# dohlee/diffab-pytorch

Hardware: NVIDIA B200
Metric: reverse-diffusion patches/s (K=128, T=100) (higher is better)
Workload: dtype bf16

## Files before the change

### diffab-pytorch_b200/csrc/ipa_sm100.cu

```cuda
#include <cuda_bf16.h>
#include <cuda_fp16.h>

#include <stdlib.h>

#include <mutex>

#include "common.cuh"
#include "gemm_sm100.cuh"
#include "ipa_proj_sm100.cuh"
#include "ipa_sm100_layout.cuh"
#include "sm100_prims.cuh"

namespace dab {

EncodeTiledFn get_encode_tiled() {
  static EncodeTiledFn fn = nullptr;
  static std::once_flag once;
  std::call_once(once, [] {
    void* p = nullptr;
    cudaDriverEntryPointQueryResult q;
    if (cudaGetDriverEntryPoint("cuTensorMapEncodeTiled", &p, cudaEnableDefault, &q) == cudaSuccess &&
        q == cudaDriverEntryPointSuccess)
      fn = reinterpret_cast<EncodeTiledFn>(p);
  });
  return fn;
}

int make_tensor_map_bf16(CUtensorMap* out, const void* base, int rank, const uint64_t* dims,
                         const uint64_t* strides_bytes, const uint32_t* box, CUtensorMapSwizzle swizzle) {
  EncodeTiledFn enc = get_encode_tiled();
  DAB_REQUIRE(enc != nullptr, DAB_ELAUNCH, "cuTensorMapEncodeTiled not available (no CUDA driver?)");
  cuuint64_t gdim[5];
  cuuint64_t gstr[5];
  cuuint32_t bdim[5], estr[5];
  for (int i = 0; i < rank; ++i) { gdim[i] = dims[i]; bdim[i] = box[i]; estr[i] = 1; }
  for (int i = 0; i + 1 < rank; ++i) gstr[i] = strides_bytes[i];
  CUresult r = enc(out, CU_TENSOR_MAP_DATA_TYPE_BFLOAT16, (cuuint32_t)rank, const_cast<void*>(base), gdim, gstr, bdim,
                   estr, CU_TENSOR_MAP_INTERLEAVE_NONE, swizzle, CU_TENSOR_MAP_L2_PROMOTION_L2_128B,
                   CU_TENSOR_MAP_FLOAT_OOB_FILL_NONE);
  DAB_REQUIRE(r == CUDA_SUCCESS, DAB_EINVAL, "cuTensorMapEncodeTiled failed with CUresult %d", (int)r);
  return DAB_OK;
}

namespace sm100 {

#ifdef DAB_DEBUG_HOOKS
static long long* g_core_dbg = nullptr;
#else
static constexpr long long* g_core_dbg = nullptr;
#endif

__global__ void __launch_bounds__(256) pack_weights_kernel(DabIpaWeights w, uint8_t* packed) {
  __shared__ float tile[32][33];
  const PackedOffsets o = packed_offsets();
  constexpr int kCatTiles = (NPROJ / 32) * (D / 32);
  const int tx = threadIdx.x & 31, ty = threadIdx.x >> 5;
  const float* src;
  __nv_bfloat16 *dst, *dst_t;
  int r0, c0, ld_src, ld_dst, ld_t, row_off = 0;
  int t = blockIdx.x;
  if (t < kCatTiles) {
    const int tr = t / (D / 32), tcn = t % (D / 32);
    r0 = tr * 32; c0 = tcn * 32;
    const float* srcs[6] = {w.w_q_scalar, w.w_k_scalar, w.w_v_scalar, w.w_q_point, w.w_k_point, w.w_v_point};
    const int seg = r0 < 3 * NS ? r0 / NS : 3 + (r0 - 3 * NS) / NPT;
    row_off = seg < 3 ? seg * NS : 3 * NS + (seg - 3) * NPT;
    src = srcs[seg]; ld_src = D;
    dst = reinterpret_cast<__nv_bfloat16*>(packed + o.wcat); ld_dst = D;
    dst_t = reinterpret_cast<__nv_bfloat16*>(packed + o.wcat_t); ld_t = NPROJ;
  } else {
    t -= kCatTiles;
    const int tr = t / (NCAT / 32), tcn = t % (NCAT / 32);
    r0 = tr * 32; c0 = tcn * 32;
    src = w.w_out; ld_src = NCAT;
    dst = reinterpret_cast<__nv_bfloat16*>(packed + o.wout); ld_dst = NCAT;
    dst_t = reinterpret_cast<__nv_bfloat16*>(packed + o.wout_t); ld_t = D;
  }
#pragma unroll
  for (int k = 0; k < 4; ++k) {
    const int r = ty + 8 * k;
    const float v = __ldg(src + (size_t)(r0 - row_off + r) * ld_src + c0 + tx);
    tile[r][tx] = v;
    dst[(size_t)(r0 + r) * ld_dst + c0 + tx] = __float2bfloat16_rn(v);
  }
  __syncthreads();
#pragma unroll
  for (int k = 0; k < 4; ++k) {
    const int c = ty + 8 * k;
    dst_t[(size_t)(c0 + c) * ld_t + r0 + tx] = __float2bfloat16_rn(tile[tx][c]);
  }
  if (blockIdx.x == 0) {
    float* wpb = reinterpret_cast<float*>(packed + o.wpb);
    for (int i = threadIdx.x; i < H * C; i += 256) wpb[i] = w.w_pair_bias[i];
    float* bout = reinterpret_cast<float*>(packed + o.bout);
    float* gam = reinterpret_cast<float*>(packed + o.gamma);
    for (int i = threadIdx.x; i < D; i += 256) bout[i] = w.b_out[i];
    for (int i = threadIdx.x; i < H; i += 256) gam[i] = w.gamma[i];
  }
}
constexpr int kPackBlocks = (NPROJ / 32) * (D / 32) + (D / 32) * (NCAT / 32);

struct CoreSmem {
  static constexpr int kSlot = L * C * 2;
  static constexpr int kSlots = 4;
  static constexpr int kRing = 0;
  static constexpr int kKBuf = 3 * L * 64;
  static constexpr int kKBufs = 3;
  static constexpr int kKRing = kRing + kSlots * kSlot;
  static constexpr int kCtx0 = kKRing + kKBufs * kKBuf;
  static constexpr int kPh = 0;
  static constexpr int kPhBytes = H * 2 * IB * 128;
  static constexpr int kQBuf = H * 3 * IB * 64;
  static constexpr int kPi = kPh + kPhBytes;
  static constexpr int kPiSlot = 2 * 2048;
  static constexpr int kCtxBytes = kPi + 2 * kPiSlot;
  static constexpr int kMisc = kCtx0 + 2 * kCtxBytes;
  static constexpr int kRedMax = kMisc;
  static constexpr int kBars = kRedMax + 2 * 1024;
  static constexpr int kNumBars = 48;
  static constexpr int kTmemSlot = kBars + kNumBars * 8;
  static constexpr int kTotal = kTmemSlot + 16;
};
static_assert(CoreSmem::kQBuf <= CoreSmem::kPhBytes, "Q must fit the idle P_h region");
static_assert(CoreSmem::kTotal <= 227 * 1024, "one CTA per SM");

enum Bar { K_FULL = 0, K_EMPTY = 3, R_FULL = 6, R_EMPTY = 10, K_TURN = 14, R_TURN = 15, CTX_BARS = 16, N_BARS = 16 + 2 * 13 };
enum CtxBar { Q_FULL = 0, S_DONE = 1, PAIR = 2 , O_DONE = 4, P_READY = 5 ,
              EPI_TMEM = 9 ,
              EPI_DONE = 10 ,
              EPI_SFREE = 11 , N_CTX_BARS = 13 };
static_assert(N_BARS <= CoreSmem::kNumBars, "barrier storage");

constexpr uint32_t kColS = 0, kColPair = 128 , kTmemCols = 512;

template <bool IS_MAX>
__device__ __forceinline__ float warp_reduce8(const float (&v)[8], int lane) {
  auto op = [](float a, float b) { return IS_MAX ? fmaxf(a, b) : a + b; };
  const bool u1 = lane & 16, u2 = lane & 8, u3 = lane & 4;
  float a[4], bq[2];
#pragma unroll
  for (int k = 0; k < 4; ++k) {
    float send = u1 ? v[k] : v[k + 4], keep = u1 ? v[k + 4] : v[k];
    a[k] = op(keep, __shfl_xor_sync(0xffffffffu, send, 16));
  }
#pragma unroll
  for (int k = 0; k < 2; ++k) {
    float send = u2 ? a[k] : a[k + 2], keep = u2 ? a[k + 2] : a[k];
    bq[k] = op(keep, __shfl_xor_sync(0xffffffffu, send, 8));
  }
  float send = u3 ? bq[0] : bq[1], keep = u3 ? bq[1] : bq[0];
  float c = op(keep, __shfl_xor_sync(0xffffffffu, send, 4));
  c = op(c, __shfl_xor_sync(0xffffffffu, c, 2));
  c = op(c, __shfl_xor_sync(0xffffffffu, c, 1));
  return c;
}

__device__ __forceinline__ float warp_reduce16_max(const float (&v)[16], int lane) {
  const bool u1 = lane & 16, u2 = lane & 8, u3 = lane & 4, u4 = lane & 2;
  float a[8], b4[4], c2[2];
#pragma unroll
  for (int k = 0; k < 8; ++k) {
    float send = u1 ? v[k] : v[k + 8], keep = u1 ? v[k + 8] : v[k];
    a[k] = fmaxf(keep, __shfl_xor_sync(0xffffffffu, send, 16));
  }
#pragma unroll
  for (int k = 0; k < 4; ++k) {
    float send = u2 ? a[k] : a[k + 4], keep = u2 ? a[k + 4] : a[k];
    b4[k] = fmaxf(keep, __shfl_xor_sync(0xffffffffu, send, 8));
  }
#pragma unroll
  for (int k = 0; k < 2; ++k) {
    float send = u3 ? b4[k] : b4[k + 2], keep = u3 ? b4[k + 2] : b4[k];
    c2[k] = fmaxf(keep, __shfl_xor_sync(0xffffffffu, send, 4));
  }
  float send = u4 ? c2[0] : c2[1], keep = u4 ? c2[1] : c2[0];
  float d = fmaxf(keep, __shfl_xor_sync(0xffffffffu, send, 2));
  return fmaxf(d, __shfl_xor_sync(0xffffffffu, d, 1));
}

__device__ __forceinline__ void tmem_ld_x4(uint32_t taddr, float (&v)[4]) {
  uint32_t r[4];
  asm volatile("tcgen05.ld.sync.aligned.32x32b.x4.b32 {%0,%1,%2,%3}, [%4];"
               : "=r"(r[0]), "=r"(r[1]), "=r"(r[2]), "=r"(r[3])
               : "r"(taddr));
#pragma unroll
  for (int i = 0; i < 4; ++i) v[i] = __uint_as_float(r[i]);
}

constexpr int kCoreThreads = 640;
template <bool KB2>
__global__ void __launch_bounds__(kCoreThreads, 1)
ipa_core_kernel(const __grid_constant__ CUtensorMap map_q, const __grid_constant__ CUtensorMap map_k,
                const __grid_constant__ CUtensorMap map_v, const __grid_constant__ CUtensorMap map_e,
                const uint4* __restrict__ bias, const float* __restrict__ tc, const float* __restrict__ R,
                __nv_bfloat16* __restrict__ cat, float* __restrict__ stats, uint4* __restrict__ pu,
                int n_tiles, long long* __restrict__ dbg, int64_t out_stride) {
  extern __shared__ __align__(1024) uint8_t smem[];
  long long* dbg_cta = nullptr;
#define DAB_STAMP(k) do { if (dbg_cta && (threadIdx.x & 255) == 0) dbg_cta[(k)] = clock64(); } while (0)
#define DAB_STAMP_ISSUER(k) do { if (dbg_cta) dbg_cta[(k)] = clock64(); } while (0)
#define DAB_TIMED_WAIT(bar, par, acc) do { if (dbg) { long long t0_ = clock64(); mbar_wait((bar), (par)); (acc) += clock64() - t0_; } else mbar_wait((bar), (par)); } while (0)
  using S = CoreSmem;
  uint64_t* bars = reinterpret_cast<uint64_t*>(smem + S::kBars);
  uint32_t* tmem_slot = reinterpret_cast<uint32_t*>(smem + S::kTmemSlot);

  const int tid = threadIdx.x, warp = tid >> 5, lane = tid & 31;
  const uint32_t smem_base = smem_u32(smem);
  if ((smem_base & 1023u) != 0) asm volatile("trap;");
  const int n_local = (n_tiles - (int)blockIdx.x + (int)gridDim.x - 1) / (int)gridDim.x;
  auto tile_of = [&](int k) { return n_tiles - 1 - ((int)blockIdx.x + k * (int)gridDim.x); };
  struct TileIdx { int64_t q0, kv0, o0; int lrow, joff; };
  auto decode = [&](int tile) {
    TileIdx ti;
    const int v = tile >> 3, it = tile & 7;
    if (KB2) {
      const int qblk = v >> 1, kb = v & 1;
      ti.q0 = (int64_t)qblk * L + it * IB;
      ti.kv0 = (int64_t)((qblk & ~1) + kb) * L;
      ti.o0 = (int64_t)kb * out_stride + ti.q0;
      ti.lrow = 2 * L; ti.joff = kb * L;
    } else {
      ti.q0 = (int64_t)v * L + it * IB; ti.kv0 = (int64_t)v * L; ti.o0 = ti.q0; ti.lrow = L; ti.joff = 0;
    }
    return ti;
  };
  auto pos_e = [](int r) { return r; };
  auto pos_v = [](int h) { return IB + h; };
  auto k_use = [](int k, int h) { return k * (h % 3 == 2 ? 2 : 3) + h / 3; };

  if (tid == 0) {
    for (int i = 0; i < CTX_BARS; ++i) mbar_init(&bars[i], 1u);
    for (int c = 0; c < 2; ++c)
      for (int i = 0; i < N_CTX_BARS; ++i)
        mbar_init(&bars[CTX_BARS + N_CTX_BARS * c + i], (i >= P_READY && i < P_READY + 4) ? 128u : (i >= EPI_TMEM ? 256u : 1u));
    fence_barrier_init();
  }
  __syncwarp();
  if (warp == 0) tmem_alloc(tmem_slot, kTmemCols);
  tcgen05_fence_before_sync();
  __syncthreads();
  tcgen05_fence_after_sync();
  const uint32_t tmem_cta = *tmem_slot;

  if (warp == 18) {
    if (lane == 0) {
      tma_prefetch_desc(&map_q); tma_prefetch_desc(&map_k);
      for (int k = 0; k < n_local; ++k) {
        const int c = k & 1, n = k >> 1, tile = tile_of(k);
        const TileIdx ti = decode(tile);
        const int64_t row0 = ti.q0;
        const int kvrow = (int)ti.kv0;
        uint64_t* cb = bars + CTX_BARS + N_CTX_BARS * c;
        uint8_t* cs = smem + S::kCtx0 + c * S::kCtxBytes;
        auto load_k = [&](int h) {
          const int s = h % S::kKBufs;
          if (k > 0 || h >= S::kKBufs) mbar_wait(&bars[K_EMPTY + s], (k_use(k, h) - 1) & 1);
          uint8_t* kb = smem + S::kKRing + s * S::kKBuf;
          mbar_arrive_expect_tx(&bars[K_FULL + s], S::kKBuf);
          for (int blk = 0; blk < 3; ++blk)
            tma_load_2d(kb + blk * (L * 64), &map_k, &bars[K_FULL + s], (h * 3 + blk) * 32, kvrow);
        };
        load_k(0);
        load_k(1);
        load_k(2);
        if (n > 0) mbar_wait(&cb[O_DONE], (n - 1) & 1);
        mbar_arrive_expect_tx(&cb[Q_FULL], S::kQBuf);
        for (int blk = 0; blk < H * 3; ++blk)
          tma_load_2d(cs + S::kPh + blk * (IB * 64), &map_q, &cb[Q_FULL], blk * 32, (int)row0);
        for (int h = S::kKBufs; h < H; ++h) load_k(h);
      }
    }
  } else if (warp == 19) {
    if (lane == 0) {
      tma_prefetch_desc(&map_v); tma_prefetch_desc(&map_e);
      const uint64_t pol = policy_evict_first();
#ifndef DAB_L2_AHEAD
#define DAB_L2_AHEAD 8
#endif
      constexpr int kL2Ahead = DAB_L2_AHEAD;
      auto pair0_of = [&](int k, int r) { const TileIdx ti = decode(tile_of(k)); return (int)((ti.q0 + r) * ti.lrow + ti.joff); };
      if (n_local > 0)
        for (int r = 0; r < kL2Ahead; ++r) tma_prefetch_l2_2d_hint(&map_e, 0, pair0_of(0, r), pol);
      for (int k = 0; k < n_local; ++k) {
        const int kvrow = (int)decode(tile_of(k)).kv0;
        const bool has_next = k + 1 < n_local;
        for (int x = 0; x < IB + H; ++x) {
          const int s = x % S::kSlots;
          if (k > 0 || x >= S::kSlots) mbar_wait(&bars[R_EMPTY + s], ((x / S::kSlots) + 1) & 1);
          mbar_arrive_expect_tx(&bars[R_FULL + s], S::kSlot);
          if (x < IB) {
            tma_load_2d_hint(smem + S::kRing + s * S::kSlot, &map_e, &bars[R_FULL + s], 0, pair0_of(k, x), pol);
            const int a = x + kL2Ahead;
            if (a < IB) tma_prefetch_l2_2d_hint(&map_e, 0, pair0_of(k, a), pol);
            else if (has_next) tma_prefetch_l2_2d_hint(&map_e, 0, pair0_of(k + 1, a - IB), pol);
          } else {
            tma_load_2d(smem + S::kRing + s * S::kSlot, &map_v, &bars[R_FULL + s], (x - IB) * V_W, kvrow);
          }
        }
      }
    }
  } else if (warp >= 16) {
    const int c = __shfl_sync(0xffffffffu, warp, 0) - 16;
    {
      constexpr uint32_t kIdescS = make_idesc_bf16(128, 16, 0, 0);
      constexpr uint32_t kIdescPair = make_idesc_bf16(128, 16, 1, 0);
      constexpr uint32_t kIdescO = make_idesc_f16(128, 32, 1, 0);
      uint64_t* cb = bars + CTX_BARS + N_CTX_BARS * c;
      const uint32_t cs = smem_base + S::kCtx0 + c * S::kCtxBytes;
      const uint32_t tmem = tmem_cta + 256u * c;
      const uint64_t dK0 = make_smem_desc(smem_base + S::kKRing, 16, 512, kSwizzle64B);
      const uint64_t dQ0 = make_smem_desc(cs + S::kPh, 16, 512, kSwizzle64B);
      const uint64_t dR0 = make_smem_desc(smem_base + S::kRing, S::kSlot, 1024, kSwizzle128B);
      const uint64_t dPi0 = make_smem_desc(cs + S::kPi, 16, 1024, kSwizzle128B);
      const uint64_t dPh0 = make_smem_desc(cs + S::kPh, 16, 1024, kSwizzle128B);
      for (int k = c, n = 0; k < n_local; k += 2, ++n) {
        dbg_cta = (dbg && lane == 0) ? dbg + (size_t)tile_of(k) * 64 : nullptr;
        long long w_q = 0, w_sfree = 0, w_kturn = 0, w_k = 0, w_epit = 0, w_rturn = 0, w_e = 0, w_p = 0, w_v = 0;
        DAB_STAMP_ISSUER(16);
        DAB_TIMED_WAIT(&cb[Q_FULL], n & 1, w_q);
        if (n > 0) {
          DAB_TIMED_WAIT(&cb[EPI_SFREE], (n - 1) & 1, w_sfree);
        }
        if (k > 0) DAB_TIMED_WAIT(&bars[K_TURN], (k - 1) & 1, w_kturn);
        tcgen05_fence_after_sync();
        DAB_STAMP_ISSUER(1);
        for (int h = 0; h < H; ++h) {
          const int s = h % S::kKBufs;
          DAB_TIMED_WAIT(&bars[K_FULL + s], k_use(k, h) & 1, w_k);
          tcgen05_fence_after_sync();
          DAB_STAMP_ISSUER(48 + h);
          if (elect_one()) {
            const uint64_t ka = dK0 + (uint32_t)((s * S::kKBuf) >> 4);
            const uint64_t qa = dQ0 + (uint32_t)((h * 3 * (IB * 64)) >> 4);
#pragma unroll
            for (int m = 0; m < 4; ++m) {
              const int ablk = (m == 0) ? 0 : (m == 3 ? 2 : 1), bblk = (m == 0) ? 0 : (m == 2 ? 2 : 1);
#pragma unroll
              for (int kk = 0; kk < 2; ++kk)
                umma_bf16(tmem + kColS + h * 16, ka + (uint32_t)((ablk * (L * 64) + kk * 32) >> 4),
                          qa + (uint32_t)((bblk * (IB * 64) + kk * 32) >> 4), kIdescS, (m | kk) != 0);
            }
            umma_commit(&bars[K_EMPTY + s]);
          }
          __syncwarp();
        }
        if (elect_one()) {
          umma_commit(&cb[S_DONE]);
          mbar_arrive(&bars[K_TURN]);
        }
        __syncwarp();
        DAB_STAMP_ISSUER(2);
        if (n > 0) DAB_TIMED_WAIT(&cb[EPI_TMEM], (n - 1) & 1, w_epit);
        if (k > 0) DAB_TIMED_WAIT(&bars[R_TURN], (k - 1) & 1, w_rturn);
        DAB_STAMP_ISSUER(17);
        for (int p = 0; p < IB / 2; ++p) {
          const int x = pos_e(2 * p), st = x % S::kSlots;
          const int slot = p & 1;
          DAB_TIMED_WAIT(&bars[R_FULL + st], (x / S::kSlots) & 1, w_e);
          DAB_TIMED_WAIT(&bars[R_FULL + st + 1], (x / S::kSlots) & 1, w_e);
          if (p == 4) DAB_STAMP_ISSUER(41);
          DAB_TIMED_WAIT(&cb[P_READY + slot], (p >> 1) & 1, w_p);
          DAB_TIMED_WAIT(&cb[P_READY + 2 + slot], (p >> 1) & 1, w_p);
          tcgen05_fence_after_sync();
          if (p == 4) DAB_STAMP_ISSUER(42);
          if (elect_one()) {
            const uint64_t ea = dR0 + (uint32_t)((st * S::kSlot) >> 4);
            const uint64_t pa = dPi0 + (uint32_t)((slot * S::kPiSlot) >> 4);
#pragma unroll
            for (int kk = 0; kk < L / 16; ++kk)
              umma_bf16(tmem + kColPair + p * 16, ea + (uint32_t)((kk * 2048) >> 4),
                        pa + (uint32_t)(((kk >> 2) * 2048 + (kk & 3) * 32) >> 4), kIdescPair, kk != 0);
            umma_commit(&cb[PAIR + slot]);
            umma_commit(&bars[R_EMPTY + st]);
            umma_commit(&bars[R_EMPTY + st + 1]);
          }
          __syncwarp();
          if (p == 4) DAB_STAMP_ISSUER(43);
        }
        DAB_STAMP_ISSUER(3);
        for (int m = 0; m < H / 2; ++m) {
          const int x = pos_v(2 * m), st = x % S::kSlots;
          DAB_TIMED_WAIT(&bars[R_FULL + st], (x / S::kSlots) & 1, w_v);
          DAB_TIMED_WAIT(&bars[R_FULL + st + 1], (x / S::kSlots) & 1, w_v);
          tcgen05_fence_after_sync();
          DAB_STAMP_ISSUER(56 + m);
          if (elect_one()) {
            const uint64_t va = dR0 + (uint32_t)((st * S::kSlot) >> 4);
            const uint64_t pa = dPh0 + (uint32_t)(((2 * m) * (IB * 128)) >> 4);
#pragma unroll
            for (int kk = 0; kk < L / 16; ++kk)
              umma_bf16(tmem + kColS + m * 32, va + (uint32_t)((kk * 2048) >> 4),
                        pa + (uint32_t)(((kk >> 2) * (H * IB * 128) + (kk & 3) * 32) >> 4), kIdescO, kk != 0);
            umma_commit(&bars[R_EMPTY + st]);
            umma_commit(&bars[R_EMPTY + st + 1]);
          }
          __syncwarp();
        }
        if (elect_one()) {
          umma_commit(&cb[O_DONE]);
          mbar_arrive(&bars[R_TURN]);
        }
        __syncwarp();
        DAB_STAMP_ISSUER(7);
        if (dbg_cta) {
          dbg_cta[18] = w_q; dbg_cta[19] = w_sfree; dbg_cta[20] = w_kturn; dbg_cta[21] = w_k; dbg_cta[22] = w_epit;
          dbg_cta[23] = w_rturn; dbg_cta[25] = w_e; dbg_cta[26] = w_p; dbg_cta[27] = w_v;
        }
      }
    }
  } else {
    const int c = warp >> 3, cw = warp & 7;
    const int g = cw >> 2, gw = cw & 3, gt = tid & 127, ct = tid & 255;
    uint64_t* cb = bars + CTX_BARS + N_CTX_BARS * c;
    uint8_t* cs = smem + S::kCtx0 + c * S::kCtxBytes;
    const uint32_t tmem = tmem_cta + 256u * c;
    const uint32_t tmem_lane = tmem + ((uint32_t)(gw * 32) << 16);
    const int vsel = ((lane >> 4) & 1) * 8 + ((lane >> 3) & 1) * 4 + ((lane >> 2) & 1) * 2 + ((lane >> 1) & 1);
    float* red_max = reinterpret_cast<float*>(smem + S::kRedMax) + c * 256 + g * 128;
    float* red_ctx = reinterpret_cast<float*>(smem + S::kRedMax) + c * 256;
    float* inv_o = red_ctx;
    auto bar_group = [&] { asm volatile("bar.sync %0, 128;" ::"r"(1 + 2 * c + g) : "memory"); };
    auto bar_all_compute = [&] { asm volatile("bar.sync %0, 256;" ::"r"(5 + c) : "memory"); };
    (void)ct;

   for (int k = c, tn = 0; k < n_local; k += 2, ++tn) {
    const int tile = tile_of(k);
    const TileIdx ti = decode(tile);
    const int64_t row0 = ti.q0;
    const int64_t orow0 = KB2 ? ti.o0 : row0;
    constexpr int64_t LR = KB2 ? 2 * L : L;
    dbg_cta = dbg ? dbg + (size_t)tile * 64 : nullptr;
    long long w_pair = 0;
    DAB_STAMP(0);
    const uint4* bias_t = bias + (row0 + g) * LR + (KB2 ? ti.joff : 0) + gt;
    uint4 b_cur[2] = {__ldg(bias_t), __ldg(bias_t + 2 * LR)};
    uint4 b_nxt[2] = {__ldg(bias_t + 4 * LR), __ldg(bias_t + 6 * LR)};
    mbar_wait(&cb[S_DONE], tn & 1);
    tcgen05_fence_after_sync();
    DAB_STAMP(6);
    for (int q = 0; q < IB / 4; ++q) {
      const uint4 b_use[2] = {b_cur[0], b_cur[1]};
      b_cur[0] = b_nxt[0]; b_cur[1] = b_nxt[1];
      if (q + 2 < IB / 4) {
        b_nxt[0] = __ldg(bias_t + (size_t)(2 * q + 4) * 2 * LR);
        b_nxt[1] = __ldg(bias_t + (size_t)(2 * q + 5) * 2 * LR);
      }
      float sreg[H][4];
#pragma unroll
      for (int h = 0; h < H; ++h) tmem_ld_x4(tmem_lane + kColS + h * 16 + 4 * q, sreg[h]);
      tmem_wait_ld();
      if (q == IB / 4 - 1) tcgen05_fence_before_sync();
      if (q == 2) DAB_STAMP(33);
      float lg[16];
#pragma unroll
      for (int r = 0; r < 2; ++r) {
        const __half2* hb = reinterpret_cast<const __half2*>(&b_use[r]);
#pragma unroll
        for (int kk = 0; kk < 4; ++kk) {
          float2 f = __half22float2(hb[kk]);
          lg[r * 8 + 2 * kk] = f.x; lg[r * 8 + 2 * kk + 1] = f.y;
        }
#pragma unroll
        for (int h = 0; h < H; ++h) {
          const float sv = g == 0 ? (r == 0 ? sreg[h][0] : sreg[h][2]) : (r == 0 ? sreg[h][1] : sreg[h][3]);
          lg[r * 8 + h] += sv;
        }
      }
      float wm = warp_reduce16_max(lg, lane);
      float* rm = red_max + (q & 1) * 64;
      if ((lane & 1) == 0) rm[gw * 16 + vsel] = wm;
      bar_group();
      if (q == 2) DAB_STAMP(34);
      float mx[16];
      {
        const float4* r4 = reinterpret_cast<const float4*>(rm);
#pragma unroll
        for (int kk = 0; kk < 4; ++kk) {
          float4 a = r4[kk], bb = r4[4 + kk], cc = r4[8 + kk], dd = r4[12 + kk];
          mx[4 * kk] = fmaxf(fmaxf(a.x, bb.x), fmaxf(cc.x, dd.x));
          mx[4 * kk + 1] = fmaxf(fmaxf(a.y, bb.y), fmaxf(cc.y, dd.y));
          mx[4 * kk + 2] = fmaxf(fmaxf(a.z, bb.z), fmaxf(cc.z, dd.z));
          mx[4 * kk + 3] = fmaxf(fmaxf(a.w, bb.w), fmaxf(cc.w, dd.w));
        }
      }
      if (stats && gt < 16) {
        float v = mx[0];
#pragma unroll
        for (int kk = 1; kk < 16; ++kk) v = (kk == gt) ? mx[kk] : v;
        stats[(orow0 + 2 * (2 * q + (gt >> 3)) + g) * 16 + (gt & 7)] = v;
      }
#pragma unroll
      for (int r = 0; r < 2; ++r) {
        const int n = 2 * q + r, i = 2 * n + g;
        float p[8];
#pragma unroll
        for (int h = 0; h < H; ++h) p[h] = ex2(lg[r * 8 + h] - mx[r * 8 + h]);
        if (pu)
          pu[(row0 + i) * L + gt] = make_uint4(pack_bf162(p[0], p[1]), pack_bf162(p[2], p[3]), pack_bf162(p[4], p[5]),
                                               pack_bf162(p[6], p[7]));
        if (n >= 2) DAB_TIMED_WAIT(&cb[PAIR + (n & 1)], ((n >> 1) - 1) & 1, w_pair);
        {
          const int je = gt & ~1;
          const uint32_t kb = je >> 6, chunk = (je & 63) >> 3, e2 = (je & 7) * 2;
          uint8_t* pi = cs + S::kPi + (n & 1) * S::kPiSlot + kb * 2048 + g * 1024;
          uint8_t* ph = cs + S::kPh + kb * (H * IB * 128);
          const bool odd = lane & 1;
#pragma unroll
          for (int hh = 0; hh < 4; ++hh) {
            float send = odd ? p[2 * hh] : p[2 * hh + 1];
            float recv = __shfl_xor_sync(0xffffffffu, send, 1);
            const int h = 2 * hh + (odd ? 1 : 0);
            float lo = odd ? recv : p[2 * hh], hi = odd ? p[2 * hh + 1] : recv;
            *reinterpret_cast<uint32_t*>(pi + swz128_offset(h, chunk) + e2) = pack_bf162(lo, hi);
            *reinterpret_cast<uint32_t*>(ph + h * (IB * 128) + swz128_offset(i, chunk) + e2) = pack_h2(lo, hi);
          }
        }
        fence_proxy_async_smem();
        tcgen05_fence_before_sync();
        mbar_arrive(&cb[P_READY + g * 2 + (n & 1)]);
        if (g == 0) DAB_STAMP(8 + n);
      }
    }
    DAB_STAMP(24);
    if (dbg_cta && (tid & 255) == 0) dbg_cta[28] = w_pair;

    float Rm[9], tfr[3];
    {
      const int64_t row = row0 + (gt >> 3);
#pragma unroll
      for (int cc = 0; cc < 9; ++cc) Rm[cc] = __ldg(R + row * 9 + cc);
#pragma unroll
      for (int cc = 0; cc < 3; ++cc) tfr[cc] = __ldg(tc + row * 3 + cc);
    }
    uint8_t* stage_e = cs + S::kPh + S::kQBuf + 12288 + cw * 512;
    mbar_wait(&cb[O_DONE], tn & 1);
    tcgen05_fence_after_sync();
    DAB_STAMP(4);
    const int hsel = gw >> 1;
    const uint32_t ocol = kColS + (uint32_t)hsel * 16;
    if (gw & 1) {
#pragma unroll
      for (int mm = 0; mm < 2; ++mm) {
        const int m = 2 * g + mm, h = 2 * m + hsel;
        float o[16];
        tmem_ld_x16(tmem_lane + ocol + m * 32, o);
        tmem_wait_ld();
        if (lane == 24) {
#pragma unroll
          for (int i = 0; i < IB; ++i) inv_o[i * H + h] = __fdividef(1.0f, o[i]);
        }
      }
    }
    bar_all_compute();
    if (stats && g == 0) stats[(orow0 + (gt >> 3)) * 16 + 8 + (gt & 7)] = inv_o[gt];
    float* s_og = reinterpret_cast<float*>(cs + S::kPh + S::kQBuf);
#pragma unroll
    for (int mm = 0; mm < 2; ++mm) {
      const int m = 2 * g + mm, h = 2 * m + hsel;
      float o[16];
      tmem_ld_x16(tmem_lane + ocol + m * 32, o);
      tmem_wait_ld();
      if ((gw & 1) == 0) {
        __nv_bfloat16* st16 = reinterpret_cast<__nv_bfloat16*>(stage_e);
#pragma unroll
        for (int r = 0; r < 2; ++r) {
#pragma unroll
          for (int i = 0; i < 8; ++i) st16[i * 32 + lane] = __float2bfloat16_rn(o[8 * r + i] * inv_o[(8 * r + i) * H + h]);
          __syncwarp();
          const int i = 8 * r + (lane >> 2), part = lane & 3;
          *reinterpret_cast<uint4*>(cat + (orow0 + i) * NCAT + h * DS + part * 8) = reinterpret_cast<const uint4*>(stage_e)[lane];
          __syncwarp();
        }
      } else if (lane < 3 * P) {
#pragma unroll
        for (int i = 0; i < IB; ++i) s_og[(i * H + h) * 24 + lane] = o[i] * inv_o[i * H + h];
      }
    }
    tcgen05_fence_before_sync();
    mbar_arrive(&cb[EPI_SFREE]);
    bar_all_compute();
    if (g == 0) {
      const int i = gt >> 3, h = gt & 7;
      const int64_t row = row0 + i;
      const float* gp = s_og + (i * H + h) * 24;
      const float tx = tfr[0], ty = tfr[1], tz = tfr[2];
      float out[24], nrm[8];
#pragma unroll
      for (int p = 0; p < P; ++p) {
        float gx = gp[3 * p] - tx, gy = gp[3 * p + 1] - ty, gz = gp[3 * p + 2] - tz;
        float lx = gx * Rm[0] + gy * Rm[1] + gz * Rm[2];
        float ly = gx * Rm[3] + gy * Rm[4] + gz * Rm[5];
        float lz = gx * Rm[6] + gy * Rm[7] + gz * Rm[8];
        out[3 * p] = lx; out[3 * p + 1] = ly; out[3 * p + 2] = lz;
        nrm[p] = sqrtf(lx * lx + ly * ly + lz * lz);
      }
      const int64_t orow = orow0 + i;
      uint4* dpt = reinterpret_cast<uint4*>(cat + orow * NCAT + NS + H * C + h * 24);
#pragma unroll
      for (int q = 0; q < 3; ++q)
        dpt[q] = make_uint4(pack_bf162(out[8 * q], out[8 * q + 1]), pack_bf162(out[8 * q + 2], out[8 * q + 3]),
                            pack_bf162(out[8 * q + 4], out[8 * q + 5]), pack_bf162(out[8 * q + 6], out[8 * q + 7]));
      *reinterpret_cast<uint4*>(cat + orow * NCAT + NS + H * C + NPT + h * 8) =
          make_uint4(pack_bf162(nrm[0], nrm[1]), pack_bf162(nrm[2], nrm[3]), pack_bf162(nrm[4], nrm[5]),
                     pack_bf162(nrm[6], nrm[7]));
    }
    for (int n = g; n < IB / 2; n += 2) {
      const int i = 2 * n + hsel;
      float v[8];
      tmem_ld_x8(tmem_lane + kColPair + n * 16 + hsel * 8, v);
      tmem_wait_ld();
      {
        const float4 a0 = *reinterpret_cast<const float4*>(inv_o + i * H), a1 = *reinterpret_cast<const float4*>(inv_o + i * H + 4);
        const float na[8] = {a0.x, a0.y, a0.z, a0.w, a1.x, a1.y, a1.z, a1.w};
        __nv_bfloat16* st16 = reinterpret_cast<__nv_bfloat16*>(stage_e);
#pragma unroll
        for (int h = 0; h < H; ++h) st16[h * 32 + lane] = __float2bfloat16_rn(v[h] * na[h]);
      }
      __syncwarp();
      {
        const int h = lane >> 2, part = lane & 3;
        *reinterpret_cast<uint4*>(cat + (orow0 + i) * NCAT + NS + h * C + (gw & 1) * 32 + part * 8) =
            reinterpret_cast<const uint4*>(stage_e)[lane];
      }
      __syncwarp();
    }
    tcgen05_fence_before_sync();
    mbar_arrive(&cb[EPI_TMEM]);
    DAB_STAMP(5);
    bar_all_compute();
   }
  }
  tcgen05_fence_before_sync();
  __syncthreads();
#undef DAB_STAMP
#undef DAB_STAMP_ISSUER
#undef DAB_TIMED_WAIT
  if (warp == 0) tmem_free(tmem_cta, kTmemCols);
}

struct BiasSmem {
  static constexpr int kStage = 128 * C * 2;
  static constexpr int kStages = 4;
  static constexpr int kW = kStages * kStage;
  static constexpr int kBars = kW + 96 * 128;
  static constexpr int kTmemSlot = kBars + 16 * 8;
  static constexpr int kTotal = kTmemSlot + 16;
};
__global__ void __launch_bounds__(192, 2)
ipa_pair_bias_mma_kernel(const __grid_constant__ CUtensorMap map_e, const float* __restrict__ wpb ,
                         int nl, uint4* __restrict__ planes, int64_t n_pairs, int n_tiles) {
  extern __shared__ __align__(1024) uint8_t smem[];
  using S = BiasSmem;
  uint64_t* bars = reinterpret_cast<uint64_t*>(smem + S::kBars);
  uint32_t* tmem_slot = reinterpret_cast<uint32_t*>(smem + S::kTmemSlot);
  const int tid = threadIdx.x, warp = tid >> 5, lane = tid & 31;
  const uint32_t smem_base = smem_u32(smem);
  if ((smem_base & 1023u) != 0) asm volatile("trap;");
  const int N = 16 * nl;
  if (tid == 0) {
    for (int i = 0; i < 8; ++i) mbar_init(&bars[i], 1);
    mbar_init(&bars[8], 1); mbar_init(&bars[9], 1);
    mbar_init(&bars[10], 128); mbar_init(&bars[11], 128);
    fence_barrier_init();
  }
  {
    const float sc = rsqrtf(3.0f) * kLog2e;
    for (int i = tid; i < 8 * nl * (C / 2); i += blockDim.x) {
      const int r = i / (C / 2), c2 = (i % (C / 2)) * 2;
      const float a = wpb[r * C + c2] * sc, bq = wpb[r * C + c2 + 1] * sc;
      const float ah = __bfloat162float(__float2bfloat16_rn(a)), bh = __bfloat162float(__float2bfloat16_rn(bq));
      *reinterpret_cast<uint32_t*>(smem + S::kW + swz128_offset(r, c2 >> 3) + (c2 & 7) * 2) = pack_bf162(ah, bh);
      *reinterpret_cast<uint32_t*>(smem + S::kW + swz128_offset(8 * nl + r, c2 >> 3) + (c2 & 7) * 2) =
          pack_bf162(a - ah, bq - bh);
    }
  }
  fence_proxy_async_smem();
  __syncwarp();
  if (warp == 0) tmem_alloc(tmem_slot, 256);
  tcgen05_fence_before_sync();
  __syncthreads();
  tcgen05_fence_after_sync();
  const uint32_t tmem = *tmem_slot;
  const int n_mine = (n_tiles - (int)blockIdx.x + (int)gridDim.x - 1) / (int)gridDim.x;
  if (warp == 4) {
    if (lane == 0) {
      tma_prefetch_desc(&map_e);
      for (int k = 0; k < n_mine; ++k) {
        const int s = k % S::kStages;
        if (k >= S::kStages) mbar_wait(&bars[4 + s], ((k / S::kStages) - 1) & 1);
        mbar_arrive_expect_tx(&bars[s], S::kStage);
        tma_load_2d(smem + s * S::kStage, &map_e, &bars[s], 0, (int)(((int64_t)blockIdx.x + (int64_t)k * gridDim.x) * 128));
      }
    }
  } else if (warp == 5) {
    if (lane == 0) {
      const uint32_t idesc = make_idesc_bf16(128, N, 0, 0);
      for (int k = 0; k < n_mine; ++k) {
        const int s = k % S::kStages, acc = k & 1;
        mbar_wait(&bars[s], (k / S::kStages) & 1);
        if (k >= 2) mbar_wait(&bars[10 + acc], ((k >> 1) - 1) & 1);
        tcgen05_fence_after_sync();
#pragma unroll
        for (int kk = 0; kk < C / 16; ++kk) {
// ... 423 lines not shown
```

Measured before the change: 1825.

## Interleave next tile's pair-bias loads with previous tile's V loads in ring

The ring producer now runs one step behind on V loads: for each tile after the first, the first half of pair-bias (E) rows is interleaved with the previous tile's V rows, and the remaining E rows follow. A new V_TURN barrier separates the two MMA issuer contexts, and R_TURN is now released after the pair MMAs instead of after the O MMAs. The aim is to let one context's pair-bias MMAs overlap with the other context's V MMAs so the shared ring and tensor core stay busy across tile boundaries. The slot-index mapping is more complex and a mismatch could deadlock or mis-order loads.

```diff
diff --git a/diffab-pytorch_b200/csrc/ipa_sm100.cu b/diffab-pytorch_b200/csrc/ipa_sm100.cu
--- a/diffab-pytorch_b200/csrc/ipa_sm100.cu
+++ b/diffab-pytorch_b200/csrc/ipa_sm100.cu
@@ -124,7 +124,8 @@
 static_assert(CoreSmem::kQBuf <= CoreSmem::kPhBytes, "Q must fit the idle P_h region");
 static_assert(CoreSmem::kTotal <= 227 * 1024, "one CTA per SM");
 
-enum Bar { K_FULL = 0, K_EMPTY = 3, R_FULL = 6, R_EMPTY = 10, K_TURN = 14, R_TURN = 15, CTX_BARS = 16, N_BARS = 16 + 2 * 13 };
+enum Bar { K_FULL = 0, K_EMPTY = 3, R_FULL = 6, R_EMPTY = 10, K_TURN = 14, R_TURN = 15, V_TURN = 16, CTX_BARS = 17,
+           N_BARS = 17 + 2 * 13 };
 enum CtxBar { Q_FULL = 0, S_DONE = 1, PAIR = 2 , O_DONE = 4, P_READY = 5 ,
               EPI_TMEM = 9 ,
               EPI_DONE = 10 ,
@@ -224,8 +225,8 @@
     }
     return ti;
   };
-  auto pos_e = [](int r) { return r; };
-  auto pos_v = [](int h) { return IB + h; };
+  auto pos_e = [](int k, int r) { return k == 0 ? r : (r < IB / 2 ? 4 * (r >> 1) + (r & 1) : IB / 2 + r); };
+  auto pos_v = [](bool last, int h) { return last ? h : 4 * (h >> 1) + 2 + (h & 1); };
   auto k_use = [](int k, int h) { return k * (h % 3 == 2 ? 2 : 3) + h / 3; };
 
   if (tid == 0) {
@@ -281,20 +282,28 @@
       auto pair0_of = [&](int k, int r) { const TileIdx ti = decode(tile_of(k)); return (int)((ti.q0 + r) * ti.lrow + ti.joff); };
       if (n_local > 0)
         for (int r = 0; r < kL2Ahead; ++r) tma_prefetch_l2_2d_hint(&map_e, 0, pair0_of(0, r), pol);
-      for (int k = 0; k < n_local; ++k) {
-        const int kvrow = (int)decode(tile_of(k)).kv0;
+      for (int k = 0; k <= n_local; ++k) {
+        const bool has_e = k < n_local, has_v = k > 0;
+        const int kvrow = has_v ? (int)decode(tile_of(k - 1)).kv0 : 0;
         const bool has_next = k + 1 < n_local;
-        for (int x = 0; x < IB + H; ++x) {
+        const int n_ent = (has_e ? IB : 0) + (has_v ? H : 0);
+        for (int x = 0; x < n_ent; ++x) {
+          int r = -1, h = -1;
+          if (!has_v) r = x;
+          else if (!has_e) h = x;
+          else if (x >= IB) r = x - IB / 2;
+          else if ((x & 3) < 2) r = 2 * (x >> 2) + (x & 1);
+          else h = 2 * (x >> 2) + (x & 1);
           const int s = x % S::kSlots;
           if (k > 0 || x >= S::kSlots) mbar_wait(&bars[R_EMPTY + s], ((x / S::kSlots) + 1) & 1);
           mbar_arrive_expect_tx(&bars[R_FULL + s], S::kSlot);
-          if (x < IB) {
-            tma_load_2d_hint(smem + S::kRing + s * S::kSlot, &map_e, &bars[R_FULL + s], 0, pair0_of(k, x), pol);
-            const int a = x + kL2Ahead;
+          if (r >= 0) {
+            tma_load_2d_hint(smem + S::kRing + s * S::kSlot, &map_e, &bars[R_FULL + s], 0, pair0_of(k, r), pol);
+            const int a = r + kL2Ahead;
             if (a < IB) tma_prefetch_l2_2d_hint(&map_e, 0, pair0_of(k, a), pol);
             else if (has_next) tma_prefetch_l2_2d_hint(&map_e, 0, pair0_of(k + 1, a - IB), pol);
           } else {
-            tma_load_2d(smem + S::kRing + s * S::kSlot, &map_v, &bars[R_FULL + s], (x - IB) * V_W, kvrow);
+            tma_load_2d(smem + S::kRing + s * S::kSlot, &map_v, &bars[R_FULL + s], h * V_W, kvrow);
           }
         }
       }
@@ -354,8 +363,9 @@
         if (k > 0) DAB_TIMED_WAIT(&bars[R_TURN], (k - 1) & 1, w_rturn);
         DAB_STAMP_ISSUER(17);
         for (int p = 0; p < IB / 2; ++p) {
-          const int x = pos_e(2 * p), st = x % S::kSlots;
+          const int x = pos_e(k, 2 * p), st = x % S::kSlots;
           const int slot = p & 1;
+          if (k > 0 && p == IB / 4 + 1) DAB_TIMED_WAIT(&bars[V_TURN], (k - 1) & 1, w_e);
           DAB_TIMED_WAIT(&bars[R_FULL + st], (x / S::kSlots) & 1, w_e);
           DAB_TIMED_WAIT(&bars[R_FULL + st + 1], (x / S::kSlots) & 1, w_e);
           if (p == 4) DAB_STAMP_ISSUER(41);
@@ -377,9 +387,12 @@
           __syncwarp();
           if (p == 4) DAB_STAMP_ISSUER(43);
         }
+        if (elect_one()) mbar_arrive(&bars[R_TURN]);
+        __syncwarp();
         DAB_STAMP_ISSUER(3);
+        const bool last = k + 1 >= n_local;
         for (int m = 0; m < H / 2; ++m) {
-          const int x = pos_v(2 * m), st = x % S::kSlots;
+          const int x = pos_v(last, 2 * m), st = x % S::kSlots;
           DAB_TIMED_WAIT(&bars[R_FULL + st], (x / S::kSlots) & 1, w_v);
           DAB_TIMED_WAIT(&bars[R_FULL + st + 1], (x / S::kSlots) & 1, w_v);
           tcgen05_fence_after_sync();
@@ -398,7 +411,7 @@
         }
         if (elect_one()) {
           umma_commit(&cb[O_DONE]);
-          mbar_arrive(&bars[R_TURN]);
+          mbar_arrive(&bars[V_TURN]);
         }
         __syncwarp();
         DAB_STAMP_ISSUER(7);
```

After: 1660 (median of 6 runs). -9.1%, worse.
